# Guoxs/DODT

Measured on AMD Instinct MI355X. Metric: frame-pairs/sec (whole node) KITTI-shape tau=2, higher is better.
Workload: dtype f32

## Files before the change

### dodt_amd/csrc/gemm.hip

```cpp
#include <cmath>
#include <cstdlib>
#include <mutex>
#include <set>
#include <type_traits>
#include <vector>

#include <algorithm>

#include "common.h"
#include "lds_dma.h"

namespace {

typedef float f32x16 __attribute__((ext_vector_type(16)));
typedef float f32x4 __attribute__((ext_vector_type(4)));

constexpr int kKAlign = 64;
constexpr int kSmallK = 16;

struct GemmArgs {
    const float* x;
    const float* x2;
    const float* w;
    const float* bias;
// ... 514 lines not shown

int launch_fc_bf16_dma(hipStream_t s, const GemmArgs& a, int Npad, bool y_bf16, int bk) {
    const int tiles_m = dodt::ceil_div(a.M, kBfBM), tiles_n = Npad / kBfBN;
    const dim3 grid(tiles_m * tiles_n);
    const size_t lds = (size_t)kBfStages * (kBfBM + kBfBN) * bk * 2;
    hipError_t e;
    if (bk == 64 && y_bf16) e = launch_with_lds(&fc_bf16_dma_kernel<true, 64>, grid, lds, s, a, tiles_m, tiles_n);
    else if (bk == 64) e = launch_with_lds(&fc_bf16_dma_kernel<false, 64>, grid, lds, s, a, tiles_m, tiles_n);
    else if (y_bf16) e = launch_with_lds(&fc_bf16_dma_kernel<true, 32>, grid, lds, s, a, tiles_m, tiles_n);
    else e = launch_with_lds(&fc_bf16_dma_kernel<false, 32>, grid, lds, s, a, tiles_m, tiles_n);
    DODT_HIP_CHECK(e);
    DODT_LAUNCH_CHECK();
    return DODT_OK;
}

int bf16_dma_bk() {
    static const int bk = getenv("DODT_FC_BF16_DMA_BK") && atoi(getenv("DODT_FC_BF16_DMA_BK")) == 64 ? 64 : 32;
    return bk;
}

struct SplitOut {
    float* y[3];
    int n_end[3];
    int ld[3];
};

__device__ __forceinline__ f32x4 mfma16x4(float a, float b, f32x4 c) {
    return __builtin_amdgcn_mfma_f32_16x16x4f32(a, b, c, 0, 0, 0);
}

typedef __bf16 bf16x4 __attribute__((ext_vector_type(4)));
typedef short s16x4 __attribute__((ext_vector_type(4)));

template <bool BF16, bool XB16 = false>
__global__ void __launch_bounds__(512)
fc_skinny_kernel(const GemmArgs a, const SplitOut so) {
    static_assert(BF16 || !XB16, "bf16 rows feed the bf16 arithmetic only");
    __shared__ f32x4 s_part[8][2][64];
    const int tid = threadIdx.x, lane = tid & 63, wave = tid >> 6;
    const int i = lane & 15, g = lane >> 4;
    const int M = resolved_rows(a.d_m, a.M);
    const int m0 = blockIdx.x * 16;
    if (m0 >= M) return;
    const float* xr = a.x + (size_t)min(m0 + i, M - 1) * a.ldx + 4 * g;
    const unsigned short* xr16 = reinterpret_cast<const unsigned short*>(a.x) + (size_t)min(m0 + i, M - 1) * a.ldx + 4 * g;
    const int steps = a.K / 16;
    f32x4 acc0 = {0.f, 0.f, 0.f, 0.f}, acc1 = {0.f, 0.f, 0.f, 0.f};
    constexpr int U = 4;
    if constexpr (BF16) {
        const f32x2* w2 = reinterpret_cast<const f32x2*>(a.w) + ((g >> 1) * 32 + i) * 2 + (g & 1);
        for (int j0 = wave; j0 < steps; j0 += 8 * U) {
            f32x4 xv[U];
            f32x2 wa[U], wb[U];
#pragma unroll
            for (int u = 0; u < U; ++u) {
                const int j = j0 + 8 * u;
                const bool ok = j < steps;
                const int jj = ok ? j : wave;
                if constexpr (XB16) {
                    const f32x2 x2 = *reinterpret_cast<const f32x2*>(xr16 + 16 * jj);
                    xv[u] = f32x4{x2[0], x2[1], 0.f, 0.f};
                } else {
                    xv[u] = *reinterpret_cast<const f32x4*>(xr + 16 * jj);
                }
                const f32x2 z = {0.f, 0.f};
                wa[u] = ok ? w2[(size_t)jj * 128] : z;
                wb[u] = ok ? w2[(size_t)jj * 128 + 32] : z;
            }
#pragma unroll
            for (int u = 0; u < U; ++u) {
                const f32x2 xb = XB16 ? f32x2{xv[u][0], xv[u][1]}
                                      : f32x2{pack_bf16(xv[u][0], xv[u][1]), pack_bf16(xv[u][2], xv[u][3])};
                acc0 = __builtin_amdgcn_mfma_f32_16x16x16bf16_1k(__builtin_bit_cast(s16x4, xb),
                                                                 __builtin_bit_cast(s16x4, wa[u]), acc0, 0, 0, 0);
                acc1 = __builtin_amdgcn_mfma_f32_16x16x16bf16_1k(__builtin_bit_cast(s16x4, xb),
                                                                 __builtin_bit_cast(s16x4, wb[u]), acc1, 0, 0, 0);
            }
        }
    } else {
        const f32x4* w4 = reinterpret_cast<const f32x4*>(a.w) + g * 32 + i;
        for (int j0 = wave; j0 < steps; j0 += 8 * U) {
            f32x4 xv[U], wa[U], wb[U];
#pragma unroll
            for (int u = 0; u < U; ++u) {
                const int j = j0 + 8 * u;
                const bool ok = j < steps;
                const int jj = ok ? j : wave;
                xv[u] = *reinterpret_cast<const f32x4*>(xr + 16 * jj);
                const f32x4 z = {0.f, 0.f, 0.f, 0.f};
                wa[u] = ok ? w4[(size_t)jj * 128] : z;
                wb[u] = ok ? w4[(size_t)jj * 128 + 16] : z;
            }
#pragma unroll
            for (int u = 0; u < U; ++u)
#pragma unroll
                for (int s = 0; s < 4; ++s) {
                    acc0 = mfma16x4(xv[u][s], wa[u][s], acc0);
                    acc1 = mfma16x4(xv[u][s], wb[u][s], acc1);
                }
        }
    }
    s_part[wave][0][lane] = acc0;
    s_part[wave][1][lane] = acc1;
    __syncthreads();
    if (tid >= 128) return;
    const int nb = tid >> 6;
    f32x4 sum = s_part[0][nb][lane];
#pragma unroll
    for (int w = 1; w < 8; ++w) sum += s_part[w][nb][lane];
    const int n = nb * 16 + i;
    if (n >= a.N) return;
    const float b = a.bias[n];
    const int p = (n >= so.n_end[0]) + (n >= so.n_end[1]);
    float* y = p == 0 ? so.y[0] : (p == 1 ? so.y[1] : so.y[2]);
    const int ld = p == 0 ? so.ld[0] : (p == 1 ? so.ld[1] : so.ld[2]);
    const int nn = n - (p == 0 ? 0 : (p == 1 ? so.n_end[0] : so.n_end[1]));
#pragma unroll
    for (int r = 0; r < 4; ++r) {
        const int m = m0 + 4 * g + r;
        if (m < M) {
            float v = sum[r] + b;
            if (a.relu) v = fmaxf(v, 0.0f);
            y[(size_t)m * ld + nn] = v;
        }
    }
}

template <bool BF16>
__global__ void __launch_bounds__(256)
fc_smallk_kernel(const GemmArgs a, const float* __restrict__ w_plain) {
    const int M = resolved_rows(a.d_m, a.M);
    const int n4 = a.N >> 2;
    const long long t = (long long)blockIdx.x * blockDim.x + threadIdx.x;
    const int m = (int)(t / n4), c = (int)(t - (long long)m * n4) * 4;
    if (m >= M) return;
    const float* x = a.x + (size_t)m * a.ldx;
    const float* x2 = a.x2 ? a.x2 + (size_t)m * a.ldx : nullptr;
    f32x4 acc = {0.f, 0.f, 0.f, 0.f};
    for (int k = 0; k < a.K; ++k) {
        float xv = x[k];
        if (x2) xv = (xv + x2[k]) / 2.0f;
        if constexpr (BF16) xv = bf16_value(pack_bf16(xv, 0.0f), 0);
        const f32x4 wv = *reinterpret_cast<const f32x4*>(w_plain + (size_t)k * a.N + c);
        acc += wv * xv;
    }
    const f32x4 b = *reinterpret_cast<const f32x4*>(a.bias + c);
    acc += b;
    if (a.relu) {
#pragma unroll
        for (int i = 0; i < 4; ++i) acc[i] = fmaxf(acc[i], 0.0f);
    }
    float* y = a.y + (size_t)m * a.ldy + c;
    if ((a.ldy & 3) == 0) *reinterpret_cast<f32x4*>(y) = acc;
    else {
#pragma unroll
        for (int i = 0; i < 4; ++i) y[i] = acc[i];
    }
}

int launch_fc_skinny(hipStream_t s, const GemmArgs& a, const SplitOut& so, bool bf16, bool x_bf16) {
    if (x_bf16) hipLaunchKernelGGL((fc_skinny_kernel<true, true>), dim3(dodt::ceil_div(a.M, 16)), dim3(512), 0, s, a, so);
    else if (bf16) hipLaunchKernelGGL(fc_skinny_kernel<true>, dim3(dodt::ceil_div(a.M, 16)), dim3(512), 0, s, a, so);
    else hipLaunchKernelGGL(fc_skinny_kernel<false>, dim3(dodt::ceil_div(a.M, 16)), dim3(512), 0, s, a, so);
    DODT_LAUNCH_CHECK();
    return DODT_OK;
}

int launch_fc_smallk(hipStream_t s, const GemmArgs& a, const float* w_plain, bool bf16) {
    const long long threads = (long long)a.M * (a.N / 4);
    const dim3 grid((unsigned)((threads + 255) / 256));
    if (bf16) hipLaunchKernelGGL(fc_smallk_kernel<true>, grid, dim3(256), 0, s, a, w_plain);
    else hipLaunchKernelGGL(fc_smallk_kernel<false>, grid, dim3(256), 0, s, a, w_plain);
    DODT_LAUNCH_CHECK();
    return DODT_OK;
}

}

namespace {
__global__ void __launch_bounds__(256)
mean_fusion_kernel(const float4* __restrict__ a, const float4* __restrict__ b, int rows, const int* __restrict__ d_n,
                   int row4, float4* __restrict__ out) {
    const int lim = d_n ? min(*d_n, rows) : rows;
    const long long total = (long long)lim * row4;
    for (long long i = (long long)blockIdx.x * blockDim.x + threadIdx.x; i < total;
         i += (long long)gridDim.x * blockDim.x) {
        const float4 x = a[i], y = b[i];
        out[i] = make_float4((x.x + y.x) / 2.0f, (x.y + y.y) / 2.0f, (x.z + y.z) / 2.0f, (x.w + y.w) / 2.0f);
    }
}
}

extern "C" int dodt_mean_fusion(dodt_ctx* ctx, const float* d_a, const float* d_b, int rows, const int32_t* d_n,
                                int row_floats, float* d_out) {
    DODT_REQUIRE(ctx && d_a && d_b && d_out, "dodt_mean_fusion: NULL argument");
    DODT_REQUIRE(rows >= 0 && row_floats >= 4 && row_floats % 4 == 0,
// ... 336 lines not shown
```

### dodt_amd/csrc/nms.hip

```cpp
#include "common.h"

namespace {

constexpr int kTile = 8192;
constexpr int kSortThreads = 1024;
constexpr int kChunkRows = 2048;
constexpr int kColGroup = 1;
constexpr int kRankMax = 32768;
constexpr int kRankSeg = 512;

struct NmsState {
    int count;
    int done;
    int n_eff;
    int pad;
};

__device__ __forceinline__ uint32_t ordered_bits(float f) {
    const uint32_t b = __float_as_uint(f);
    return (b & 0x80000000u) ? ~b : (b | 0x80000000u);
}

__global__ void __launch_bounds__(256)
nms_keys_kernel(const float* __restrict__ scores, int n, const int* __restrict__ d_n, int n_pad,
// ... 168 lines not shown
    unsigned long long words[kColGroup];
#pragma unroll
    for (int g = 0; g < kColGroup; ++g) {
        const int cb = cb0 + g;
        unsigned long long mine = 0ull;
        if (cb >= rb && cb < nb) {
            const int col = cb * 64 + lane;
            float cy0 = 0, cx0 = 0, cy1 = 0, cx1 = 0, ca = -1.0f;
            if (col < n_eff) {
                const float* p = sb + (size_t)col * 5;
                cy0 = p[0]; cx0 = p[1]; cy1 = p[2]; cx1 = p[3]; ca = p[4];
            }
            unsigned long long hits = 0ull;
            for (int r = 0; r < 64; ++r) {
                const float* q = s_rows[wave][r];
                const bool hit = (col > rb * 64 + r) &&
                                 iou_gt(q[0], q[1], q[2], q[3], q[4], cy0, cx0, cy1, cx1, ca, thr);
                const unsigned long long w = __ballot(hit);
                if (lane == r) mine = w;
                hits |= hit ? (1ull << r) : 0ull;
            }
            if (cb == rb) diag_cols[col] = hits;
        }
        words[g] = mine;
    }
    if (row < n_eff) {
        unsigned long long* o = mask + (size_t)(row - row0) * nb + cb0;
#pragma unroll
        for (int g = 0; g < kColGroup; ++g)
            if (cb0 + g < nb) o[g] = words[g];
    }
}

constexpr int kScanDepth = 4;

__global__ void __launch_bounds__(1024)
nms_scan_kernel(const unsigned long long* __restrict__ mask,
                const unsigned long long* __restrict__ diag_cols, const int* __restrict__ sorted_idx,
                NmsState* __restrict__ st, unsigned long long* __restrict__ g_removed, int row0,
                int rows, int nb, int max_out, int* __restrict__ sel_out,
                int* __restrict__ count_out, int last_chunk) {
    extern __shared__ __attribute__((aligned(16))) unsigned long long s_dyn[];
    unsigned long long* const s_removed = s_dyn;
    unsigned long long* const s_cols = s_dyn + nb;
    unsigned long long* const s_kept = s_cols + rows;
    __shared__ unsigned long long s_sel;
    __shared__ int s_count, s_done;
    const int tid = threadIdx.x, lane = tid & 63, wave = tid >> 6;
    const int n_eff = st->n_eff;
    if (st->done) {
        if (last_chunk && tid == 0) *count_out = st->count;
        return;
    }
    const int b0 = row0 >> 6;
    const int b1 = min((row0 + rows + 63) >> 6, (n_eff + 63) >> 6);
    auto load_block = [&](int b, unsigned long long (&v)[4]) {
        const int c = b + 1 + lane;
        const bool ok = b < b1 && c < b1;
        const unsigned long long* base = mask + (size_t)(b * 64 - row0 + wave) * nb + c;
#pragma unroll
        for (int k = 0; k < 4; ++k) v[k] = ok ? base[(size_t)(16 * k) * nb] : 0ull;
    };
    unsigned long long v[kScanDepth][4];
#pragma unroll
    for (int d = 0; d < kScanDepth - 1; ++d) load_block(b0 + d, v[d]);
    for (int c = tid; c < nb; c += 1024) s_removed[c] = g_removed[c];
    for (int r = tid; r < (b1 - b0) * 64; r += 1024) s_cols[r] = diag_cols[b0 * 64 + r];
    if (tid < b1 - b0) s_kept[tid] = 0ull;
    if (tid == 0) { s_count = st->count; s_done = 0; }
    __syncthreads();

    auto block = [&](auto stage, int b) -> bool {
        constexpr int S = decltype(stage)::value;
        load_block(b + kScanDepth - 1, v[(S + kScanDepth - 1) % kScanDepth]);
        if (tid < 64) {
            const int row = b * 64 + lane;
            const unsigned long long cols = s_cols[(b - b0) * 64 + lane];
            const int valid = min(64, n_eff - b * 64);
            unsigned long long init = ~s_removed[b];
            if (valid < 64) init &= (1ull << valid) - 1ull;
            const bool mine = (init >> lane) & 1ull;
            unsigned long long alive = __ballot(mine);
            for (;;) {
                const unsigned long long na = __ballot(mine && (cols & alive) == 0ull);
                if (na == alive) break;
                alive = na;
            }
            const int cnt0 = __builtin_amdgcn_readfirstlane(s_count);
            const int room = max_out - cnt0;
            const unsigned long long below = (1ull << lane) - 1ull;
            unsigned long long sel = alive;
            if (__popcll(sel) > room)
                sel = __ballot(((sel >> lane) & 1ull) && __popcll(sel & below) < room);
            const int cnt = cnt0 + __popcll(sel);
            if ((sel >> lane) & 1ull) sel_out[cnt0 + __popcll(sel & below)] = sorted_idx[row];
            if (lane == 0) {
                s_sel = sel;
                s_kept[b - b0] = sel;
                s_count = cnt;
                if (cnt >= max_out) s_done = 1;
            }
        }
        __syncthreads();
        const unsigned long long sel = s_sel;
        const bool done = s_done != 0;
        if (!done && sel != 0ull) {
            unsigned long long acc = 0ull;
#pragma unroll
            for (int k = 0; k < 4; ++k)
                if ((sel >> (wave + 16 * k)) & 1ull) acc |= v[S][k];
            if (acc) atomicOr(&s_removed[b + 1 + lane], acc);
        }
        __syncthreads();
        return done;
    };
    bool stop = false;
    for (int b = b0; b < b1 && !stop; b += kScanDepth) {
        stop = block(std::integral_constant<int, 0>{}, b);
        if (!stop && b + 1 < b1) stop = block(std::integral_constant<int, 1>{}, b + 1);
        if (!stop && b + 2 < b1) stop = block(std::integral_constant<int, 2>{}, b + 2);
        if (!stop && b + 3 < b1) stop = block(std::integral_constant<int, 3>{}, b + 3);
    }
    static_assert(kScanDepth == 4, "the loop above is unrolled by hand");

    if (!stop && row0 + rows < n_eff) {
        const int nrows = (b1 - b0) * 64;
        for (int ct = b1; ct < nb; ct += 64) {
            const int c = ct + lane;
            if (c >= nb) continue;
            const unsigned long long* base = mask + (size_t)(b0 * 64 - row0) * nb + c;
            unsigned long long acc = 0ull;
            for (int r0 = wave; r0 < nrows; r0 += 16 * 8) {
                unsigned long long w[8];
#pragma unroll
                for (int k = 0; k < 8; ++k) w[k] = base[(size_t)min(r0 + 16 * k, nrows - 1) * nb];
#pragma unroll
                for (int k = 0; k < 8; ++k) {
                    const int r = r0 + 16 * k;
                    if (r < nrows && ((s_kept[r >> 6] >> (r & 63)) & 1ull)) acc |= w[k];
                }
            }
            if (acc) atomicOr(&s_removed[c], acc);
        }
        __syncthreads();
    }
    for (int c = tid; c < nb; c += 1024) g_removed[c] = s_removed[c];
    if (tid == 0) {
        st->count = s_count;
        const int exhausted = (row0 + rows >= n_eff);
        if (s_done || exhausted) st->done = 1;
        if (last_chunk || s_done || exhausted) *count_out = s_count;
    }
}

int next_pow2(int v) {
    int p = 1;
    while (p < v) p <<= 1;
    return p;
}

struct NmsPlan {
    int n_pad, nb, n_rows;
    bool ranked;
    int sort_tiles;
    int first_rows, later_rows, chunk_rows, n_chunks;
    size_t o_state, o_keys, o_rank, o_sb, o_idx, o_removed, o_diag, o_mask, scratch_bytes;
    size_t scan_lds;
    int rows_at(int row0) const {
        const int want = row0 == 0 ? first_rows : later_rows;
        return (n_rows - row0) < want ? (n_rows - row0) : want;
    }
};

NmsPlan plan_nms(int n, int max_out) {
    NmsPlan p;
    p.n_pad = next_pow2(n < 2 ? 2 : n);
    p.nb = dodt::ceil_div(n, 64);
    p.n_rows = p.nb * 64;
    p.ranked = n <= kRankMax;
// ... 86 lines not shown
        DODT_LAUNCH_CHECK();
        hipLaunchKernelGGL(nms_scatter_kernel, dim3(dodt::ceil_div(n_rows, 256)), dim3(256), 0, s,
                           d_boxes, rank, st, n_rows, sb, sorted_idx);
        DODT_LAUNCH_CHECK();
    } else {
        const int tile = n_pad / p.sort_tiles;
        hipLaunchKernelGGL(nms_sort_local, dim3(p.sort_tiles), dim3(kSortThreads), (size_t)tile * 8, s,
                           keys, n_pad);
        DODT_LAUNCH_CHECK();
        for (int k = 2 * kTile; k <= n_pad; k <<= 1) {
            for (int j = k >> 1; j >= kTile; j >>= 1) {
                hipLaunchKernelGGL(nms_sort_global_step, dim3(dodt::ceil_div(n_pad / 2, 256)),
                                   dim3(256), 0, s, keys, n_pad, k, j);
                DODT_LAUNCH_CHECK();
            }
            hipLaunchKernelGGL(nms_sort_local_merge, dim3(n_pad / kTile), dim3(kSortThreads),
                               (size_t)kTile * 8, s, keys, n_pad, k);
            DODT_LAUNCH_CHECK();
        }
        hipLaunchKernelGGL(nms_gather_kernel, dim3(dodt::ceil_div(n_rows, 256)), dim3(256), 0, s,
                           d_boxes, keys, st, n_rows, sb, sorted_idx);
        DODT_LAUNCH_CHECK();
    }
    const int col_groups = dodt::ceil_div(nb, kColGroup);
    static const hipError_t lds_attr = hipFuncSetAttribute(
        reinterpret_cast<const void*>(nms_scan_kernel), hipFuncAttributeMaxDynamicSharedMemorySize, 128 * 1024);
    DODT_HIP_CHECK(lds_attr);
    for (int row0 = 0; row0 < n_rows;) {
        const int rows = p.rows_at(row0);
        hipLaunchKernelGGL(nms_mask_kernel, dim3(col_groups, dodt::ceil_div(rows / 64, 4)),
                           dim3(256), 0, s, sb, st, row0, rows, nb, iou_threshold, mask, diag_cols);
        DODT_LAUNCH_CHECK();
        const int last = (row0 + rows >= n_rows);
        hipLaunchKernelGGL(nms_scan_kernel, dim3(1), dim3(1024), p.scan_lds, s, mask, diag_cols,
                           sorted_idx, st, removed, row0, rows, nb, max_out, d_sel_out,
                           d_count_out, last);
        DODT_LAUNCH_CHECK();
        row0 += rows;
    }
    return DODT_OK;
}
```

### dodt_amd/csrc/conv_variants.h

```cpp
#pragma once
#include <vector>

#include "conv_kernels.h"
#include "wino_kernels.h"
#include "wino43_kernel.h"
#include "deconv_kernel.h"
#include "conv_bf16_dma.h"

namespace dodt {

enum class Family {
    Direct,
    SmallCin,
    Wino22,
    Wino43,
    DeconvDma,
    Bf16Dma,
    Bf16Stream,
    Bf16First2,
};

struct KernelVariant {
    int TW, MTB, WM, WN, BN, CK;
    bool deconv;
// ... 28 lines not shown
    return v;
}

template <int TW, int MTB, int WM, int WN, int BN, bool DECONV, bool BF16 = false, int PARTS = 1>
struct Inst {
    using Cfg = ConvCfg<TW, MTB, WM, WN, BN, DECONV, PARTS>;
    static_assert(Cfg::kLdsBytes <= 160 * 1024, "variant does not fit the LDS");
    static void launch(const ConvArgs& a, dim3 grid, hipStream_t s) {
        hipLaunchKernelGGL((conv3x3_mfma_kernel<TW, MTB, WM, WN, BN, DECONV, BF16, PARTS>), grid,
                           dim3(256), Cfg::kLdsBytes, s, a);
    }
    static hipError_t prepare() {
        return hipFuncSetAttribute(
            reinterpret_cast<const void*>(&conv3x3_mfma_kernel<TW, MTB, WM, WN, BN, DECONV, BF16, PARTS>),
            hipFuncAttributeMaxDynamicSharedMemorySize, Cfg::kLdsBytes);
    }
    static KernelVariant variant() {
        int per_cu = Cfg::kMinWaves;
        const int by_lds = (160 * 1024) / Cfg::kLdsBytes;
        if (per_cu > by_lds) per_cu = by_lds;
        KernelVariant v{TW, MTB, WM, WN, BN, BF16 ? 16 : kCK, DECONV, Family::Direct, Cfg::TH,
                        Cfg::kLdsBytes, per_cu, &launch, &prepare};
        v.bf16 = BF16;
        v.parts = PARTS;
        return v;
    }
};

template <int TB, int CB>
struct InstWino {
    using Cfg = WinoCfg<TB, CB>;
    static_assert(Cfg::kLdsBytes <= 160 * 1024, "variant does not fit the LDS");
    static void launch(const ConvArgs& a, dim3 grid, hipStream_t s) {
        hipLaunchKernelGGL((wino3x3_f32_kernel<TB, CB>), grid, dim3(256), Cfg::kLdsBytes, s, a);
    }
    static hipError_t prepare() {
        return hipFuncSetAttribute(reinterpret_cast<const void*>(&wino3x3_f32_kernel<TB, CB>),
                                   hipFuncAttributeMaxDynamicSharedMemorySize, Cfg::kLdsBytes);
    }
    static KernelVariant variant() {
        return KernelVariant{Cfg::TW, 0, 4, 1, Cfg::BN, kCK, false, Family::Wino22, Cfg::TH, Cfg::kLdsBytes,
                             2, &launch, &prepare};
    }
};

struct InstWino43 {
    using Cfg = Wino43Cfg;
    static_assert(Cfg::kLdsBytes <= 160 * 1024, "variant does not fit the LDS");
    static void launch(const ConvArgs& a, dim3 grid, hipStream_t s) {
        hipLaunchKernelGGL(wino43_f32_kernel<0>, grid, dim3(256), Cfg::kLdsBytes, s, a);
    }
    static hipError_t prepare() {
        return hipFuncSetAttribute(reinterpret_cast<const void*>(&wino43_f32_kernel<0>),
                                   hipFuncAttributeMaxDynamicSharedMemorySize, Cfg::kLdsBytes);
    }
    static KernelVariant variant() {
        return KernelVariant{Cfg::TW, 0, 4, 1, Cfg::BN, kCK, false, Family::Wino43, Cfg::TH, Cfg::kLdsBytes, 1,
                             &launch, &prepare};
    }
};

template <int CB, bool BF16 = false>
struct InstDeconvDma {
    using Cfg = DeconvCfg<CB>;
    static void launch(const ConvArgs& a, dim3 grid, hipStream_t s) {
        hipLaunchKernelGGL((deconv3x3_dma_kernel<CB, BF16>), grid, dim3(256), Cfg::kLdsBytes, s, a);
    }
    static hipError_t prepare() {
        return hipFuncSetAttribute(reinterpret_cast<const void*>(&deconv3x3_dma_kernel<CB, BF16>),
// ... 98 lines not shown
```

### dodt_amd/csrc/wino_kernels.h

```cpp
#pragma once
#include <hip/hip_runtime.h>

#include <type_traits>

#include "conv_kernels.h"
#include "lds_dma.h"

namespace dodt {

typedef float f32x2_t __attribute__((ext_vector_type(2)));

template <int TB, int CB>
struct WinoCfg {
    static_assert(TB * CB == 2, "128 accumulator registers per wave");
    static constexpr int TW = 16;
    static constexpr int TH = 16 * TB;
    static constexpr int BN = 16 * CB;
    static constexpr int PH = TH + 2, PW = TW + 2;
    static constexpr int kPitch = PW + 1;
    static constexpr int kPatchSlots = (PH * kPitch + 1) * 2;
    static constexpr int kPatchInstr = (kPatchSlots + 63) / 64;
    static constexpr int kPatchFloats = kPatchInstr * 64 * 4;
    static constexpr int kWFloats = 16 * 8 * BN;
    static constexpr int kWInstr = kWFloats / 256;
    static constexpr int kBufFloats = kPatchFloats + kWFloats;
    static constexpr int kLdsBytes = 2 * kBufFloats * 4 + 16 + 1024;
    static constexpr int kInstr = kPatchInstr + kWInstr;
    static constexpr int kPerWave = (kInstr + 3) / 4;
    static constexpr int kPatchPerWave = (kPatchInstr + 3) / 4;
};

typedef float wino_f32x2 __attribute__((ext_vector_type(2)));
__device__ __forceinline__ wino_f32x2 pk_sub(wino_f32x2 a, wino_f32x2 b) {
    wino_f32x2 r;
    asm("v_pk_add_f32 %0, %1, %2 neg_lo:[0,1] neg_hi:[0,1]" : "=v"(r) : "v"(a), "v"(b));
    return r;
}

__device__ __forceinline__ f32x4 mfma16(float a, float b, f32x4 c) {
    return __builtin_amdgcn_mfma_f32_16x16x4f32(a, b, c, 0, 0, 0);
}


template <int TB, int CB>
__global__ void __launch_bounds__(256, 2)
wino3x3_f32_kernel(const ConvArgs a) {
    using Cfg = WinoCfg<TB, CB>;
    constexpr int BN = Cfg::BN, PW = Cfg::PW;
    extern __shared__ __attribute__((aligned(16))) float smem[];
    int* s_ctrl = reinterpret_cast<int*>(smem + 2 * Cfg::kBufFloats);
    float* const sDummy = smem + 2 * Cfg::kBufFloats + 4;

    const int tid = threadIdx.x;
    const int lane = tid & 63;
    const int wave = __builtin_amdgcn_readfirstlane(tid >> 6);
    const int t = lane & 15, g = lane >> 4;
    const int nchunks = a.Cin / 8;
    const int in_plane = a.H * a.W * 8;

    struct Item { int frame, ntile, ty0, tx0; };
    auto decode = [&](int it) {
        const int4 v = a.items[__builtin_amdgcn_readfirstlane(it)];
        return Item{v.x, v.y, v.z, v.w};
    };

    int p_off[Cfg::kPatchPerWave];
    i32x4_t in_rsrc, w_rsrc;
    const int plane_bytes = in_plane * 4;
    auto setup_patch = [&](const Item& it) {
#pragma unroll
        for (int k = 0; k < Cfg::kPatchPerWave; ++k) {
            const int j = wave + 4 * k;
            const int s = j * 64 + lane;
            const int q = s >> 1;
            const int py = q / Cfg::kPitch;
            const int px = q - py * Cfg::kPitch - ((py >> 1) & 1);
            const int half = (s & 1) ^ ((px >> 3) & 1);
            const int gy = it.ty0 - 1 + py, gx = it.tx0 - 1 + px;
            const bool ok = j < Cfg::kPatchInstr && py < Cfg::PH && px >= 0 && px < PW &&
                            gy >= 0 && gy < a.H && gx >= 0 && gx < a.W;
// ... 38 lines not shown
            const unsigned dst = real ? lds0 + (unsigned)(2 * Cfg::kPatchFloats + img * Cfg::kWFloats + j * 256) * 4 : lds_dummy;
            blds16s(w_rsrc, real ? w_voff : kOob, wch * (Cfg::kWFloats * 4) + j * 1024, dst);
        }
    };

    const int n_items = a.n_items_dev ? *a.n_items_dev : a.n_items;
    const bool grouped = a.xcd_counters != nullptr;
    const int vx = grouped ? (int)(blockIdx.x & 7) : 0;
    const int q_lo = grouped ? vx * (n_items / 8) + min(vx, n_items % 8) : 0;
    const int q_hi = grouped ? q_lo + n_items / 8 + (vx < n_items % 8 ? 1 : 0) : n_items;
    const int q_first = q_lo + (grouped ? ((int)gridDim.x - vx + 7) / 8 : (int)gridDim.x);
    int* const q_counter = grouped ? a.xcd_counters + 16 * vx : a.counter;
    int comp_item = q_lo + (grouped ? (int)(blockIdx.x >> 3) : (int)blockIdx.x);
    if (comp_item >= q_hi) return;
    int q0 = n_items;
    auto advance = [&](int& it, int& ch, bool patch) {
        if (it >= n_items) return;
        if (++ch == nchunks) {
            ch = 0;
            it = (it == comp_item) ? q0 : n_items;
            if (it < n_items) {
                if (patch) setup_patch(decode(it));
                else setup_w(decode(it));
            } else if (patch) {
                in_rsrc[2] = 0;
            } else {
                w_rsrc[2] = 0;
            }
        }
    };

    const int tyl = t >> 3, txl = t & 7;
    const int w_lane = (g * (CB / 2) * 16 + t) * 4;
    int row_off[TB][4], col_off[4];
#pragma unroll
    for (int c = 0; c < 4; ++c) {
        const int px = 2 * txl + c;
        col_off[c] = px * 8 + (((g >> 1) ^ ((px >> 3) & 1)) * 4) + (g & 1) * 2;
    }
#pragma unroll
    for (int tb = 0; tb < TB; ++tb)
#pragma unroll
        for (int r = 0; r < 4; ++r) {
            const int py = 2 * (2 * (wave * TB + tb) + tyl) + r;
            row_off[tb][r] = (py * Cfg::kPitch + ((py >> 1) & 1)) * 8;
        }

    auto load_d = [&](f32x2_t (&d)[4][4], int tb, int r, int pb) {
#pragma unroll
        for (int c = 0; c < 4; ++c)
            d[r][c] = *reinterpret_cast<const f32x2_t*>(sPB + pb * Cfg::kPatchFloats +
                                                          row_off[tb][r] + col_off[c]);
    };
    auto rows_d = [&](f32x2_t (&d)[4][4], int c) {
        const f32x2_t t0 = d[0][c] - d[2][c], t1 = d[1][c] + d[2][c];
        const f32x2_t t2 = d[2][c] - d[1][c], t3 = d[1][c] - d[3][c];
        d[0][c] = t0; d[1][c] = t1; d[2][c] = t2; d[3][c] = t3;
    };
    auto cols_d = [&](const f32x2_t (&d)[4][4], f32x2_t (&v)[16], int i) {
        v[i * 4 + 0] = d[i][0] - d[i][2];
        v[i * 4 + 1] = d[i][1] + d[i][2];
        v[i * 4 + 2] = d[i][2] - d[i][1];
        v[i * 4 + 3] = d[i][1] - d[i][3];
    };

    pit = wit = comp_item;
    setup_patch(decode(pit));
    setup_w(decode(wit));
#pragma unroll
    for (int n = 0; n < Cfg::kPatchPerWave; ++n) copy_n(n, 0, 0);
    advance(pit, pch, true);
#pragma unroll
    for (int n = Cfg::kPatchPerWave; n < kCopies; ++n) copy_n(n, 0, 0);
    advance(wit, wch, false);
    __builtin_amdgcn_s_waitcnt(0);
    __syncthreads();

    int k_stamp = 0;
    auto step = [&](auto par, f32x4 (&acc)[TB][CB][16], int comp_ch) {
        constexpr int PAR = decltype(par)::value;
        if (comp_ch == 0 && tid == 0) {
            const int t = q_first + atomicAdd(q_counter, 1);
            s_ctrl[0] = t < q_hi ? t : n_items;
        }
        const float* sW = sWB + PAR * Cfg::kWFloats + w_lane;
        f32x2_t d[4][4], v[16];
        const bool stamp = (a.debug & 32) && blockIdx.x == 1 && tid == 0 && k_stamp < 12;
        int* stamps = a.counter_base + 32 + (k_stamp < 12 ? k_stamp : 0) * 6;
        if (stamp) {
            stamps[0] = (int)__builtin_amdgcn_s_memtime();
            if (k_stamp == 0 || k_stamp == 11)
                a.counter_base[32 + 72 + (k_stamp != 0)] = (int)__builtin_amdgcn_s_memrealtime();
        }
        if (stamp) stamps[1] = (int)__builtin_amdgcn_s_memtime();
#pragma unroll
        for (int tb = 0; tb < TB; ++tb) {
#pragma unroll
            for (int r = 0; r < 4; ++r) load_d(d, tb, r, PAR);
#pragma unroll
            for (int c = 0; c < 4; ++c) rows_d(d, c);
#pragma unroll
            for (int i = 0; i < 4; ++i) cols_d(d, v, i);
            if (stamp) {
                stamps[2] = (int)__builtin_amdgcn_s_memtime() + (v[15][1] == 12345.f);
            }
            constexpr int kWAhead = 2;
            f32x4 wq[kWAhead + 1][CB / 2];
#pragma unroll
            for (int i = 0; i < kWAhead; ++i)
#pragma unroll
                for (int cp = 0; cp < CB / 2; ++cp)
                    wq[i][cp] = *reinterpret_cast<const f32x4*>(sW + (i * 4 * (CB / 2) + cp) * 64);
#pragma unroll
            for (int x = 0; x < 16; ++x) {
                if (x + kWAhead < 16) {
#pragma unroll
                    for (int cp = 0; cp < CB / 2; ++cp)
                        wq[(x + kWAhead) % (kWAhead + 1)][cp] =
                            *reinterpret_cast<const f32x4*>(sW + ((x + kWAhead) * 4 * (CB / 2) + cp) * 64);
                }
                __builtin_amdgcn_sched_barrier(0);
#pragma unroll
                for (int s2 = 0; s2 < 2; ++s2)
#pragma unroll
                    for (int cb = 0; cb < CB; ++cb)
                        acc[tb][cb][x] = mfma16(wq[x % (kWAhead + 1)][cb >> 1][(cb & 1) * 2 + s2], v[x][s2],
                                                acc[tb][cb][x]);
                if (tb == 0 && x < kCopies && !(a.debug & 2)) copy_s(x, PAR ^ 1);
                __builtin_amdgcn_sched_barrier(0);
            }
        }
        if (stamp) stamps[3] = (int)__builtin_amdgcn_s_memtime();
        __builtin_amdgcn_s_waitcnt(0);
        if (stamp) stamps[4] = (int)__builtin_amdgcn_s_memtime();
        __builtin_amdgcn_s_barrier();
        if (stamp) stamps[5] = (int)__builtin_amdgcn_s_memtime();
        ++k_stamp;
        if (comp_ch == 0) q0 = s_ctrl[0];
        advance(pit, pch, true);
        advance(wit, wch, false);
    };

    while (comp_item < n_items) {
        f32x4 acc[TB][CB][16];
#pragma unroll
        for (int tb = 0; tb < TB; ++tb)
#pragma unroll
            for (int cb = 0; cb < CB; ++cb)
#pragma unroll
                for (int x = 0; x < 16; ++x) acc[tb][cb][x] = f32x4{0.f, 0.f, 0.f, 0.f};

        for (int comp_ch = 0; comp_ch < nchunks; comp_ch += 2) {
            step(std::integral_constant<int, 0>{}, acc, comp_ch);
            step(std::integral_constant<int, 1>{}, acc, comp_ch + 1);
        }

        if (!(a.debug & 1)) {
            typedef const ConvArgs __attribute__((address_space(4))) KernArgs;
            KernArgs* ep_ = (KernArgs*)__builtin_amdgcn_kernarg_segment_ptr();
            asm volatile("" : "+s"(ep_));
            KernArgs& e = *ep_;
            const Item it = decode(comp_item);
            float* out = e.out + (size_t)it.frame * e.out_frame_stride;
            const int out_rows = e.H - e.out_y0;
            const long long plane = (long long)out_rows * e.W * 8;
            const bool pool = e.pool_out != nullptr;
            const long long pplane = (long long)(e.H >> 1) * (e.W >> 1) * 8;
            const bool interior = it.ty0 + Cfg::TH <= e.H && it.tx0 + Cfg::TW <= e.W && it.ty0 >= e.out_y0;
            const float relu_floor = e.relu ? 0.0f : -__builtin_inff();
            typedef wino_f32x2 f32x2;
#pragma unroll
            for (int tb = 0; tb < TB; ++tb) {
                const int oy0 = it.ty0 + 2 * (2 * (wave * TB + tb) + tyl);
                const int ox0 = it.tx0 + 2 * txl;
                const int w8 = e.W * 8;
                const int cell = (g >> 1) * (int)plane + ((oy0 - e.out_y0) * e.W + ox0) * 8 + 4 * (g & 1);
                const int pcell = (g >> 1) * (int)pplane + ((oy0 >> 1) * (e.W >> 1) + (ox0 >> 1)) * 8 + 4 * (g & 1);
                float dot[4] = {0.f, 0.f, 0.f, 0.f};
#pragma unroll
                for (int cb = 0; cb < CB; ++cb) {
                    const int c0 = it.ntile * BN + cb * 16 + 4 * g;
                    const f32x4 sc = *reinterpret_cast<const f32x4*>(e.scale + c0);
                    const f32x4 sh = *reinterpret_cast<const f32x4*>(e.shift + c0);
                    f32x4 y[4];
#pragma unroll
                    for (int hf = 0; hf < 2; ++hf) {
                        auto M = [&](int x) { return f32x2{acc[tb][cb][x][2 * hf], acc[tb][cb][x][2 * hf + 1]}; };
                        f32x2 z[4][2];
#pragma unroll
                        for (int i = 0; i < 4; ++i) {
// ... 75 lines not shown
```

Measured before the change: 420.3.

## Shrink skinny FC and NMS scan blocks to 256 threads with more per-wave work

The skinny FC kernel now runs 4 waves instead of 8. Each wave walks two K-slices and keeps two accumulator pairs, and the per-wave unroll is reduced. The single-block NMS scan kernel drops from 1024 to 256 threads. Each wave handles 16 mask rows, uses wave-uniform scalar row addressing, and loads only one block ahead instead of a 4-deep pipeline. The intent is cheaper barriers and lower launch and occupancy cost in these latency-bound kernels, at the risk of less memory-level parallelism and a shallower prefetch.

```diff
diff --git a/dodt_amd/csrc/gemm.hip b/dodt_amd/csrc/gemm.hip
--- a/dodt_amd/csrc/gemm.hip
+++ b/dodt_amd/csrc/gemm.hip
@@ -570,8 +570,16 @@
 typedef __bf16 bf16x4 __attribute__((ext_vector_type(4)));
 typedef short s16x4 __attribute__((ext_vector_type(4)));
 
+constexpr int kSkinnyThreads = 256;
+constexpr int kSkinnyGroup = 4;
+
+__device__ __forceinline__ int skinny_walk(int steps, int t) {
+    const int own = t < steps ? (steps - t + 7) / 8 : 0;
+    return (own + kSkinnyGroup - 1) / kSkinnyGroup * kSkinnyGroup;
+}
+
 template <bool BF16, bool XB16 = false>
-__global__ void __launch_bounds__(512)
+__global__ void __launch_bounds__(kSkinnyThreads) __attribute__((amdgpu_waves_per_eu(8, 8)))
 fc_skinny_kernel(const GemmArgs a, const SplitOut so) {
     static_assert(BF16 || !XB16, "bf16 rows feed the bf16 arithmetic only");
     __shared__ f32x4 s_part[8][2][64];
@@ -583,63 +591,92 @@
     const float* xr = a.x + (size_t)min(m0 + i, M - 1) * a.ldx + 4 * g;
     const unsigned short* xr16 = reinterpret_cast<const unsigned short*>(a.x) + (size_t)min(m0 + i, M - 1) * a.ldx + 4 * g;
     const int steps = a.K / 16;
-    f32x4 acc0 = {0.f, 0.f, 0.f, 0.f}, acc1 = {0.f, 0.f, 0.f, 0.f};
-    constexpr int U = 4;
+    f32x4 acc[2][2] = {};
+    const int walk0 = skinny_walk(steps, wave), walk1 = skinny_walk(steps, wave + 4);
+    constexpr int U = BF16 ? 2 : 1;
+    static_assert(kSkinnyGroup % U == 0, "a group of steps is a whole number of batches");
     if constexpr (BF16) {
         const f32x2* w2 = reinterpret_cast<const f32x2*>(a.w) + ((g >> 1) * 32 + i) * 2 + (g & 1);
-        for (int j0 = wave; j0 < steps; j0 += 8 * U) {
-            f32x4 xv[U];
-            f32x2 wa[U], wb[U];
-#pragma unroll
-            for (int u = 0; u < U; ++u) {
-                const int j = j0 + 8 * u;
-                const bool ok = j < steps;
-                const int jj = ok ? j : wave;
-                if constexpr (XB16) {
-                    const f32x2 x2 = *reinterpret_cast<const f32x2*>(xr16 + 16 * jj);
-                    xv[u] = f32x4{x2[0], x2[1], 0.f, 0.f};
-                } else {
-                    xv[u] = *reinterpret_cast<const f32x4*>(xr + 16 * jj);
+        for (int m0 = 0; m0 < walk0; m0 += U) {
+            const int tiles = m0 < walk1 ? 2 : 1;
+            f32x4 xv[2][U];
+            f32x2 wa[2][U], wb[2][U];
+#pragma unroll
+            for (int p = 0; p < 2; ++p) {
+                if (p < tiles) {
+                    const int t = wave + 4 * p;
+#pragma unroll
+                    for (int u = 0; u < U; ++u) {
+                        const int j = t + 8 * (m0 + u);
+                        const bool ok = j < steps;
+                        const int jj = ok ? j : t;
+                        if constexpr (XB16) {
+                            const f32x2 x2 = *reinterpret_cast<const f32x2*>(xr16 + 16 * jj);
+                            xv[p][u] = f32x4{x2[0], x2[1], 0.f, 0.f};
+                        } else {
+                            xv[p][u] = *reinterpret_cast<const f32x4*>(xr + 16 * jj);
+                        }
+                        const f32x2 z = {0.f, 0.f};
+                        wa[p][u] = ok ? w2[(size_t)jj * 128] : z;
+                        wb[p][u] = ok ? w2[(size_t)jj * 128 + 32] : z;
+                    }
                 }
-                const f32x2 z = {0.f, 0.f};
-                wa[u] = ok ? w2[(size_t)jj * 128] : z;
-                wb[u] = ok ? w2[(size_t)jj * 128 + 32] : z;
-            }
-#pragma unroll
-            for (int u = 0; u < U; ++u) {
-                const f32x2 xb = XB16 ? f32x2{xv[u][0], xv[u][1]}
-                                      : f32x2{pack_bf16(xv[u][0], xv[u][1]), pack_bf16(xv[u][2], xv[u][3])};
-                acc0 = __builtin_amdgcn_mfma_f32_16x16x16bf16_1k(__builtin_bit_cast(s16x4, xb),
-                                                                 __builtin_bit_cast(s16x4, wa[u]), acc0, 0, 0, 0);
-                acc1 = __builtin_amdgcn_mfma_f32_16x16x16bf16_1k(__builtin_bit_cast(s16x4, xb),
-                                                                 __builtin_bit_cast(s16x4, wb[u]), acc1, 0, 0, 0);
+            }
+#pragma unroll
+            for (int p = 0; p < 2; ++p) {
+                if (p < tiles) {
+#pragma unroll
+                    for (int u = 0; u < U; ++u) {
+                        const f32x2 xb = XB16 ? f32x2{xv[p][u][0], xv[p][u][1]}
+                                              : f32x2{pack_bf16(xv[p][u][0], xv[p][u][1]), pack_bf16(xv[p][u][2], xv[p][u][3])};
+                        acc[p][0] = __builtin_amdgcn_mfma_f32_16x16x16bf16_1k(
+                            __builtin_bit_cast(s16x4, xb), __builtin_bit_cast(s16x4, wa[p][u]), acc[p][0], 0, 0, 0);
+                        acc[p][1] = __builtin_amdgcn_mfma_f32_16x16x16bf16_1k(
+                            __builtin_bit_cast(s16x4, xb), __builtin_bit_cast(s16x4, wb[p][u]), acc[p][1], 0, 0, 0);
+                    }
+                }
             }
         }
     } else {
         const f32x4* w4 = reinterpret_cast<const f32x4*>(a.w) + g * 32 + i;
-        for (int j0 = wave; j0 < steps; j0 += 8 * U) {
-            f32x4 xv[U], wa[U], wb[U];
-#pragma unroll
-            for (int u = 0; u < U; ++u) {
-                const int j = j0 + 8 * u;
-                const bool ok = j < steps;
-                const int jj = ok ? j : wave;
-                xv[u] = *reinterpret_cast<const f32x4*>(xr + 16 * jj);
-                const f32x4 z = {0.f, 0.f, 0.f, 0.f};
-                wa[u] = ok ? w4[(size_t)jj * 128] : z;
-                wb[u] = ok ? w4[(size_t)jj * 128 + 16] : z;
-            }
-#pragma unroll
-            for (int u = 0; u < U; ++u)
-#pragma unroll
-                for (int s = 0; s < 4; ++s) {
-                    acc0 = mfma16x4(xv[u][s], wa[u][s], acc0);
-                    acc1 = mfma16x4(xv[u][s], wb[u][s], acc1);
+        for (int m0 = 0; m0 < walk0; m0 += U) {
+            const int tiles = m0 < walk1 ? 2 : 1;
+            f32x4 xv[2][U], wa[2][U], wb[2][U];
+#pragma unroll
+            for (int p = 0; p < 2; ++p) {
+                if (p < tiles) {
+                    const int t = wave + 4 * p;
+#pragma unroll
+                    for (int u = 0; u < U; ++u) {
+                        const int j = t + 8 * (m0 + u);
+                        const bool ok = j < steps;
+                        const int jj = ok ? j : t;
+                        xv[p][u] = *reinterpret_cast<const f32x4*>(xr + 16 * jj);
+                        const f32x4 z = {0.f, 0.f, 0.f, 0.f};
+                        wa[p][u] = ok ? w4[(size_t)jj * 128] : z;
+                        wb[p][u] = ok ? w4[(size_t)jj * 128 + 16] : z;
+                    }
                 }
-        }
-    }
-    s_part[wave][0][lane] = acc0;
-    s_part[wave][1][lane] = acc1;
+            }
+#pragma unroll
+            for (int p = 0; p < 2; ++p) {
+                if (p < tiles) {
+#pragma unroll
+                    for (int u = 0; u < U; ++u)
+#pragma unroll
+                        for (int s = 0; s < 4; ++s) {
+                            acc[p][0] = mfma16x4(xv[p][u][s], wa[p][u][s], acc[p][0]);
+                            acc[p][1] = mfma16x4(xv[p][u][s], wb[p][u][s], acc[p][1]);
+                        }
+                }
+            }
+        }
+    }
+#pragma unroll
+    for (int p = 0; p < 2; ++p) {
+        s_part[wave + 4 * p][0][lane] = acc[p][0];
+        s_part[wave + 4 * p][1][lane] = acc[p][1];
+    }
     __syncthreads();
     if (tid >= 128) return;
     const int nb = tid >> 6;
@@ -697,9 +734,10 @@
 }
 
 int launch_fc_skinny(hipStream_t s, const GemmArgs& a, const SplitOut& so, bool bf16, bool x_bf16) {
-    if (x_bf16) hipLaunchKernelGGL((fc_skinny_kernel<true, true>), dim3(dodt::ceil_div(a.M, 16)), dim3(512), 0, s, a, so);
-    else if (bf16) hipLaunchKernelGGL(fc_skinny_kernel<true>, dim3(dodt::ceil_div(a.M, 16)), dim3(512), 0, s, a, so);
-    else hipLaunchKernelGGL(fc_skinny_kernel<false>, dim3(dodt::ceil_div(a.M, 16)), dim3(512), 0, s, a, so);
+    const dim3 grid(dodt::ceil_div(a.M, 16)), block(kSkinnyThreads);
+    if (x_bf16) hipLaunchKernelGGL((fc_skinny_kernel<true, true>), grid, block, 0, s, a, so);
+    else if (bf16) hipLaunchKernelGGL(fc_skinny_kernel<true>, grid, block, 0, s, a, so);
+    else hipLaunchKernelGGL(fc_skinny_kernel<false>, grid, block, 0, s, a, so);
     DODT_LAUNCH_CHECK();
     return DODT_OK;
 }
diff --git a/dodt_amd/csrc/nms.hip b/dodt_amd/csrc/nms.hip
--- a/dodt_amd/csrc/nms.hip
+++ b/dodt_amd/csrc/nms.hip
@@ -224,9 +224,17 @@
     }
 }
 
-constexpr int kScanDepth = 4;
-
-__global__ void __launch_bounds__(1024)
+__device__ __forceinline__ size_t uniform_index(size_t i) {
+    const unsigned lo = __builtin_amdgcn_readfirstlane((unsigned)i);
+    const unsigned hi = __builtin_amdgcn_readfirstlane((unsigned)(i >> 32));
+    return ((size_t)hi << 32) | lo;
+}
+
+constexpr int kScanThreads = 256;
+constexpr int kScanWaves = kScanThreads / 64;
+constexpr int kScanRows = 64 / kScanWaves;
+
+__global__ void __launch_bounds__(kScanThreads) __attribute__((amdgpu_waves_per_eu(8, 8)))
 nms_scan_kernel(const unsigned long long* __restrict__ mask,
                 const unsigned long long* __restrict__ diag_cols, const int* __restrict__ sorted_idx,
                 NmsState* __restrict__ st, unsigned long long* __restrict__ g_removed, int row0,
@@ -238,7 +246,8 @@
     unsigned long long* const s_kept = s_cols + rows;
     __shared__ unsigned long long s_sel;
     __shared__ int s_count, s_done;
-    const int tid = threadIdx.x, lane = tid & 63, wave = tid >> 6;
+    const int tid = threadIdx.x, lane = tid & 63;
+    const int wave = __builtin_amdgcn_readfirstlane(tid >> 6);
     const int n_eff = st->n_eff;
     if (st->done) {
         if (last_chunk && tid == 0) *count_out = st->count;
@@ -246,25 +255,24 @@
     }
     const int b0 = row0 >> 6;
     const int b1 = min((row0 + rows + 63) >> 6, (n_eff + 63) >> 6);
-    auto load_block = [&](int b, unsigned long long (&v)[4]) {
-        const int c = b + 1 + lane;
-        const bool ok = b < b1 && c < b1;
-        const unsigned long long* base = mask + (size_t)(b * 64 - row0 + wave) * nb + c;
-#pragma unroll
-        for (int k = 0; k < 4; ++k) v[k] = ok ? base[(size_t)(16 * k) * nb] : 0ull;
+    unsigned long long v[kScanRows] = {};
+    auto load_block = [&](int b) {
+        const unsigned off = (unsigned)min(b + 1 + lane, b1 - 1) * 8u;
+#pragma unroll
+        for (int k = 0; k < kScanRows; ++k) {
+            const unsigned long long* row = mask + uniform_index((size_t)(b * 64 - row0 + wave + kScanWaves * k) * nb);
+            v[k] = *reinterpret_cast<const unsigned long long*>(reinterpret_cast<const char*>(row) + off);
+        }
     };
-    unsigned long long v[kScanDepth][4];
-#pragma unroll
-    for (int d = 0; d < kScanDepth - 1; ++d) load_block(b0 + d, v[d]);
-    for (int c = tid; c < nb; c += 1024) s_removed[c] = g_removed[c];
-    for (int r = tid; r < (b1 - b0) * 64; r += 1024) s_cols[r] = diag_cols[b0 * 64 + r];
+    if (b0 < b1) load_block(b0);
+    for (int c = tid; c < nb; c += kScanThreads) s_removed[c] = g_removed[c];
+    for (int r = tid; r < (b1 - b0) * 64; r += kScanThreads) s_cols[r] = diag_cols[b0 * 64 + r];
     if (tid < b1 - b0) s_kept[tid] = 0ull;
     if (tid == 0) { s_count = st->count; s_done = 0; }
     __syncthreads();
 
-    auto block = [&](auto stage, int b) -> bool {
-        constexpr int S = decltype(stage)::value;
-        load_block(b + kScanDepth - 1, v[(S + kScanDepth - 1) % kScanDepth]);
+    bool stop = false;
+    for (int b = b0; b < b1 && !stop; ++b) {
         if (tid < 64) {
             const int row = b * 64 + lane;
             const unsigned long long cols = s_cols[(b - b0) * 64 + lane];
@@ -295,40 +303,34 @@
         }
         __syncthreads();
         const unsigned long long sel = s_sel;
-        const bool done = s_done != 0;
-        if (!done && sel != 0ull) {
-            unsigned long long acc = 0ull;
-#pragma unroll
-            for (int k = 0; k < 4; ++k)
-                if ((sel >> (wave + 16 * k)) & 1ull) acc |= v[S][k];
-            if (acc) atomicOr(&s_removed[b + 1 + lane], acc);
-        }
+        stop = s_done != 0;
+        if (!stop) {
+            if (sel != 0ull) {
+                unsigned long long acc = 0ull;
+#pragma unroll
+                for (int k = 0; k < kScanRows; ++k)
+                    acc |= ((sel >> (wave + kScanWaves * k)) & 1ull) ? v[k] : 0ull;
+                if (acc && b + 1 + lane < b1) atomicOr(&s_removed[b + 1 + lane], acc);
+            }
+        }
+        load_block(min(b + 1, b1 - 1));
         __syncthreads();
-        return done;
-    };
-    bool stop = false;
-    for (int b = b0; b < b1 && !stop; b += kScanDepth) {
-        stop = block(std::integral_constant<int, 0>{}, b);
-        if (!stop && b + 1 < b1) stop = block(std::integral_constant<int, 1>{}, b + 1);
-        if (!stop && b + 2 < b1) stop = block(std::integral_constant<int, 2>{}, b + 2);
-        if (!stop && b + 3 < b1) stop = block(std::integral_constant<int, 3>{}, b + 3);
-    }
-    static_assert(kScanDepth == 4, "the loop above is unrolled by hand");
+    }
 
     if (!stop && row0 + rows < n_eff) {
         const int nrows = (b1 - b0) * 64;
         for (int ct = b1; ct < nb; ct += 64) {
             const int c = ct + lane;
             if (c >= nb) continue;
-            const unsigned long long* base = mask + (size_t)(b0 * 64 - row0) * nb + c;
+            const unsigned long long* base = mask + (size_t)(b0 * 64 - row0) * nb;
             unsigned long long acc = 0ull;
-            for (int r0 = wave; r0 < nrows; r0 += 16 * 8) {
+            for (int r0 = wave; r0 < nrows; r0 += kScanWaves * 8) {
                 unsigned long long w[8];
 #pragma unroll
-                for (int k = 0; k < 8; ++k) w[k] = base[(size_t)min(r0 + 16 * k, nrows - 1) * nb];
+                for (int k = 0; k < 8; ++k) w[k] = (base + (size_t)min(r0 + kScanWaves * k, nrows - 1) * nb)[c];
 #pragma unroll
                 for (int k = 0; k < 8; ++k) {
-                    const int r = r0 + 16 * k;
+                    const int r = r0 + kScanWaves * k;
                     if (r < nrows && ((s_kept[r >> 6] >> (r & 63)) & 1ull)) acc |= w[k];
                 }
             }
@@ -336,7 +338,7 @@
         }
         __syncthreads();
     }
-    for (int c = tid; c < nb; c += 1024) g_removed[c] = s_removed[c];
+    for (int c = tid; c < nb; c += kScanThreads) g_removed[c] = s_removed[c];
     if (tid == 0) {
         st->count = s_count;
         const int exhausted = (row0 + rows >= n_eff);
@@ -489,7 +491,7 @@
                            dim3(256), 0, s, sb, st, row0, rows, nb, iou_threshold, mask, diag_cols);
         DODT_LAUNCH_CHECK();
         const int last = (row0 + rows >= n_rows);
-        hipLaunchKernelGGL(nms_scan_kernel, dim3(1), dim3(1024), p.scan_lds, s, mask, diag_cols,
+        hipLaunchKernelGGL(nms_scan_kernel, dim3(1), dim3(kScanThreads), p.scan_lds, s, mask, diag_cols,
                            sorted_idx, st, removed, row0, rows, nb, max_out, d_sel_out,
                            d_count_out, last);
         DODT_LAUNCH_CHECK();
```

Result: no change. 419.0 (-0.3%).

## Hand-schedule LDS reads in Winograd kernel and split diagnostics into separate instantiation

Applied to the files above, without the earlier changes.

Replaces compiler-generated LDS loads in the Winograd F(2,3) f32 kernel with inline-asm ds_read_b64/b128 that use precomputed addresses and constant offsets, plus explicit lgkmcnt waits. This lets the input transform start on column 0 while later columns and weight fragments are still in flight. Debug timestamp and debug-flag branches move into a kDiag template instance, so the default kernel carries no stamp code. The weight prefetch is also reduced to one b128 per point, with a static_assert restricting the kernel to TB=1, CB=2, and the first two chunk steps are peeled out of the loop. Hand-written waitcnt counts are fragile: a wrong count would silently read stale data.

```diff
diff --git a/dodt_amd/csrc/conv_variants.h b/dodt_amd/csrc/conv_variants.h
--- a/dodt_amd/csrc/conv_variants.h
+++ b/dodt_amd/csrc/conv_variants.h
@@ -84,9 +84,15 @@
     using Cfg = WinoCfg<TB, CB>;
     static_assert(Cfg::kLdsBytes <= 160 * 1024, "variant does not fit the LDS");
     static void launch(const ConvArgs& a, dim3 grid, hipStream_t s) {
-        hipLaunchKernelGGL((wino3x3_f32_kernel<TB, CB>), grid, dim3(256), Cfg::kLdsBytes, s, a);
-    }
-    static hipError_t prepare() {
+        if (conv_switches().debug || conv_switches().stamp_layer)
+            hipLaunchKernelGGL((wino3x3_f32_kernel<TB, CB, true>), grid, dim3(256), Cfg::kLdsBytes, s, a);
+        else
+            hipLaunchKernelGGL((wino3x3_f32_kernel<TB, CB>), grid, dim3(256), Cfg::kLdsBytes, s, a);
+    }
+    static hipError_t prepare() {
+        const hipError_t e = hipFuncSetAttribute(reinterpret_cast<const void*>(&wino3x3_f32_kernel<TB, CB, true>),
+                                                 hipFuncAttributeMaxDynamicSharedMemorySize, Cfg::kLdsBytes);
+        if (e != hipSuccess) return e;
         return hipFuncSetAttribute(reinterpret_cast<const void*>(&wino3x3_f32_kernel<TB, CB>),
                                    hipFuncAttributeMaxDynamicSharedMemorySize, Cfg::kLdsBytes);
     }
diff --git a/dodt_amd/csrc/wino_kernels.h b/dodt_amd/csrc/wino_kernels.h
--- a/dodt_amd/csrc/wino_kernels.h
+++ b/dodt_amd/csrc/wino_kernels.h
@@ -41,11 +41,24 @@
     return __builtin_amdgcn_mfma_f32_16x16x4f32(a, b, c, 0, 0, 0);
 }
 
-
-template <int TB, int CB>
+__device__ __forceinline__ void lds_read64(wino_f32x2& d, int off, unsigned addr) {
+    asm volatile("ds_read_b64 %0, %1 offset:%2" : "=v"(d) : "v"(addr), "n"(off));
+}
+__device__ __forceinline__ void lds_read128(f32x4& d, int off, unsigned addr) {
+    asm volatile("ds_read_b128 %0, %1 offset:%2" : "=v"(d) : "v"(addr), "n"(off));
+}
+__device__ __forceinline__ void wait_lgkm(int n, wino_f32x2& a, wino_f32x2& b, wino_f32x2& c, wino_f32x2& d) {
+    asm volatile("s_waitcnt lgkmcnt(%4)" : "+v"(a), "+v"(b), "+v"(c), "+v"(d) : "n"(n));
+}
+__device__ __forceinline__ void wait_lgkm(int n, f32x4& a) {
+    asm volatile("s_waitcnt lgkmcnt(%1)" : "+v"(a) : "n"(n));
+}
+
+template <int TB, int CB, bool kDiag = false>
 __global__ void __launch_bounds__(256, 2)
 wino3x3_f32_kernel(const ConvArgs a) {
     using Cfg = WinoCfg<TB, CB>;
+    static_assert(TB == 1 && CB == 2, "one weight fragment (ds_read_b128) per point, 14 LDS reads in flight");
     constexpr int BN = Cfg::BN, PW = Cfg::PW;
     extern __shared__ __attribute__((aligned(16))) float smem[];
     int* s_ctrl = reinterpret_cast<int*>(smem + 2 * Cfg::kBufFloats);
@@ -150,37 +163,21 @@
 
     const int tyl = t >> 3, txl = t & 7;
     const int w_lane = (g * (CB / 2) * 16 + t) * 4;
-    int row_off[TB][4], col_off[4];
-#pragma unroll
-    for (int c = 0; c < 4; ++c) {
-        const int px = 2 * txl + c;
-        col_off[c] = px * 8 + (((g >> 1) ^ ((px >> 3) & 1)) * 4) + (g & 1) * 2;
-    }
+    constexpr int kRowBytes = Cfg::kPitch * 32, kImgBytes = Cfg::kPatchFloats * 4;
+    const unsigned w_addr = lds0 + (unsigned)(2 * Cfg::kPatchFloats + w_lane) * 4;
+    unsigned tap[TB][2][4];
 #pragma unroll
     for (int tb = 0; tb < TB; ++tb)
 #pragma unroll
-        for (int r = 0; r < 4; ++r) {
-            const int py = 2 * (2 * (wave * TB + tb) + tyl) + r;
-            row_off[tb][r] = (py * Cfg::kPitch + ((py >> 1) & 1)) * 8;
-        }
-
-    auto load_d = [&](f32x2_t (&d)[4][4], int tb, int r, int pb) {
-#pragma unroll
-        for (int c = 0; c < 4; ++c)
-            d[r][c] = *reinterpret_cast<const f32x2_t*>(sPB + pb * Cfg::kPatchFloats +
-                                                          row_off[tb][r] + col_off[c]);
-    };
-    auto rows_d = [&](f32x2_t (&d)[4][4], int c) {
-        const f32x2_t t0 = d[0][c] - d[2][c], t1 = d[1][c] + d[2][c];
-        const f32x2_t t2 = d[2][c] - d[1][c], t3 = d[1][c] - d[3][c];
-        d[0][c] = t0; d[1][c] = t1; d[2][c] = t2; d[3][c] = t3;
-    };
-    auto cols_d = [&](const f32x2_t (&d)[4][4], f32x2_t (&v)[16], int i) {
-        v[i * 4 + 0] = d[i][0] - d[i][2];
-        v[i * 4 + 1] = d[i][1] + d[i][2];
-        v[i * 4 + 2] = d[i][2] - d[i][1];
-        v[i * 4 + 3] = d[i][1] - d[i][3];
-    };
+        for (int rh = 0; rh < 2; ++rh)
+#pragma unroll
+            for (int c = 0; c < 4; ++c) {
+                const int py = 2 * (2 * (wave * TB + tb) + tyl) + 2 * rh;
+                const int px = 2 * txl + c;
+                const int row_off = (py * Cfg::kPitch + ((py >> 1) & 1)) * 8;
+                const int col_off = px * 8 + (((g >> 1) ^ ((px >> 3) & 1)) * 4) + (g & 1) * 2;
+                tap[tb][rh][c] = lds0 + (unsigned)(row_off + col_off) * 4;
+            }
 
     pit = wit = comp_item;
     setup_patch(decode(pit));
@@ -201,58 +198,85 @@
             const int t = q_first + atomicAdd(q_counter, 1);
             s_ctrl[0] = t < q_hi ? t : n_items;
         }
-        const float* sW = sWB + PAR * Cfg::kWFloats + w_lane;
-        f32x2_t d[4][4], v[16];
-        const bool stamp = (a.debug & 32) && blockIdx.x == 1 && tid == 0 && k_stamp < 12;
-        int* stamps = a.counter_base + 32 + (k_stamp < 12 ? k_stamp : 0) * 6;
-        if (stamp) {
-            stamps[0] = (int)__builtin_amdgcn_s_memtime();
-            if (k_stamp == 0 || k_stamp == 11)
-                a.counter_base[32 + 72 + (k_stamp != 0)] = (int)__builtin_amdgcn_s_memrealtime();
-        }
-        if (stamp) stamps[1] = (int)__builtin_amdgcn_s_memtime();
+        bool stamp = false;
+        int* stamps = nullptr;
+        if constexpr (kDiag) {
+            stamp = (a.debug & 32) && blockIdx.x == 1 && tid == 0 && k_stamp < 12;
+            stamps = a.counter_base + 32 + (k_stamp < 12 ? k_stamp : 0) * 6;
+            if (stamp) {
+                stamps[0] = (int)__builtin_amdgcn_s_memtime();
+                if (k_stamp == 0 || k_stamp == 11)
+                    a.counter_base[32 + 72 + (k_stamp != 0)] = (int)__builtin_amdgcn_s_memrealtime();
+                stamps[1] = (int)__builtin_amdgcn_s_memtime();
+            }
+        }
 #pragma unroll
         for (int tb = 0; tb < TB; ++tb) {
-#pragma unroll
-            for (int r = 0; r < 4; ++r) load_d(d, tb, r, PAR);
-#pragma unroll
-            for (int c = 0; c < 4; ++c) rows_d(d, c);
-#pragma unroll
-            for (int i = 0; i < 4; ++i) cols_d(d, v, i);
-            if (stamp) {
-                stamps[2] = (int)__builtin_amdgcn_s_memtime() + (v[15][1] == 12345.f);
-            }
-            constexpr int kWAhead = 2;
-            f32x4 wq[kWAhead + 1][CB / 2];
-#pragma unroll
-            for (int i = 0; i < kWAhead; ++i)
-#pragma unroll
-                for (int cp = 0; cp < CB / 2; ++cp)
-                    wq[i][cp] = *reinterpret_cast<const f32x4*>(sW + (i * 4 * (CB / 2) + cp) * 64);
+            typedef wino_f32x2 f32x2;
+            f32x2 d[4][4], v[16];
+            f32x4 wq[3];
+            constexpr int kW = PAR * Cfg::kWFloats * 4;
+            auto read_col = [&](int c) {
+                lds_read64(d[0][c], PAR * kImgBytes, tap[tb][0][c]);
+                lds_read64(d[1][c], PAR * kImgBytes + kRowBytes, tap[tb][0][c]);
+                lds_read64(d[2][c], PAR * kImgBytes, tap[tb][1][c]);
+                lds_read64(d[3][c], PAR * kImgBytes + kRowBytes, tap[tb][1][c]);
+            };
+            auto rows_d = [&](int c) {
+                const f32x2 t0 = d[0][c] - d[2][c], t1 = d[1][c] + d[2][c];
+                const f32x2 t2 = d[2][c] - d[1][c], t3 = d[1][c] - d[3][c];
+                d[0][c] = t0; d[1][c] = t1; d[2][c] = t2; d[3][c] = t3;
+            };
+            auto cols_d = [&](int i) {
+                v[i * 4 + 0] = d[i][0] - d[i][2];
+                v[i * 4 + 1] = d[i][1] + d[i][2];
+                v[i * 4 + 2] = d[i][2] - d[i][1];
+                v[i * 4 + 3] = d[i][1] - d[i][3];
+            };
+            read_col(0);
+            read_col(1);
+            read_col(2);
+            wait_lgkm(8, d[0][0], d[1][0], d[2][0], d[3][0]);
+            rows_d(0);
+            read_col(3);
+            lds_read128(wq[0], kW, w_addr);
+            lds_read128(wq[1], kW + 1024, w_addr);
+            wait_lgkm(10, d[0][1], d[1][1], d[2][1], d[3][1]);
+            rows_d(1);
+            wait_lgkm(6, d[0][2], d[1][2], d[2][2], d[3][2]);
+            rows_d(2);
+            wait_lgkm(2, d[0][3], d[1][3], d[2][3], d[3][3]);
+            rows_d(3);
+#pragma unroll
+            for (int i = 0; i < 4; ++i) cols_d(i);
+            if constexpr (kDiag) {
+                if (stamp) stamps[2] = (int)__builtin_amdgcn_s_memtime() + (v[15][1] == 12345.f);
+            }
 #pragma unroll
             for (int x = 0; x < 16; ++x) {
-                if (x + kWAhead < 16) {
-#pragma unroll
-                    for (int cp = 0; cp < CB / 2; ++cp)
-                        wq[(x + kWAhead) % (kWAhead + 1)][cp] =
-                            *reinterpret_cast<const f32x4*>(sW + ((x + kWAhead) * 4 * (CB / 2) + cp) * 64);
+                if (x + 2 < 16) lds_read128(wq[(x + 2) % 3], kW + (x + 2) * 1024, w_addr);
+                wait_lgkm(x < 14 ? 2 : 15 - x, wq[x % 3]);
+                __builtin_amdgcn_sched_barrier(0);
+#pragma unroll
+                for (int s2 = 0; s2 < 2; ++s2)
+#pragma unroll
+                    for (int cb = 0; cb < CB; ++cb)
+                        acc[tb][cb][x] = mfma16(wq[x % 3][(cb & 1) * 2 + s2], v[x][s2], acc[tb][cb][x]);
+                if (tb == 0 && x < kCopies) {
+                    if constexpr (kDiag) {
+                        if (!(a.debug & 2)) copy_s(x, PAR ^ 1);
+                    } else {
+                        copy_s(x, PAR ^ 1);
+                    }
                 }
                 __builtin_amdgcn_sched_barrier(0);
-#pragma unroll
-                for (int s2 = 0; s2 < 2; ++s2)
-#pragma unroll
-                    for (int cb = 0; cb < CB; ++cb)
-                        acc[tb][cb][x] = mfma16(wq[x % (kWAhead + 1)][cb >> 1][(cb & 1) * 2 + s2], v[x][s2],
-                                                acc[tb][cb][x]);
-                if (tb == 0 && x < kCopies && !(a.debug & 2)) copy_s(x, PAR ^ 1);
-                __builtin_amdgcn_sched_barrier(0);
-            }
-        }
-        if (stamp) stamps[3] = (int)__builtin_amdgcn_s_memtime();
+            }
+        }
+        if constexpr (kDiag) { if (stamp) stamps[3] = (int)__builtin_amdgcn_s_memtime(); }
         __builtin_amdgcn_s_waitcnt(0);
-        if (stamp) stamps[4] = (int)__builtin_amdgcn_s_memtime();
+        if constexpr (kDiag) { if (stamp) stamps[4] = (int)__builtin_amdgcn_s_memtime(); }
         __builtin_amdgcn_s_barrier();
-        if (stamp) stamps[5] = (int)__builtin_amdgcn_s_memtime();
+        if constexpr (kDiag) { if (stamp) stamps[5] = (int)__builtin_amdgcn_s_memtime(); }
         ++k_stamp;
         if (comp_ch == 0) q0 = s_ctrl[0];
         advance(pit, pch, true);
@@ -268,12 +292,14 @@
 #pragma unroll
                 for (int x = 0; x < 16; ++x) acc[tb][cb][x] = f32x4{0.f, 0.f, 0.f, 0.f};
 
-        for (int comp_ch = 0; comp_ch < nchunks; comp_ch += 2) {
+        step(std::integral_constant<int, 0>{}, acc, 0);
+        step(std::integral_constant<int, 1>{}, acc, 1);
+        for (int comp_ch = 2; comp_ch < nchunks; comp_ch += 2) {
             step(std::integral_constant<int, 0>{}, acc, comp_ch);
             step(std::integral_constant<int, 1>{}, acc, comp_ch + 1);
         }
 
-        if (!(a.debug & 1)) {
+        if (!kDiag || !(a.debug & 1)) {
             typedef const ConvArgs __attribute__((address_space(4))) KernArgs;
             KernArgs* ep_ = (KernArgs*)__builtin_amdgcn_kernarg_segment_ptr();
             asm volatile("" : "+s"(ep_));
```

Result: faster. 420.8 before, 438.0 after, median of 6 (+4.1%).
